# PABannier/bark.cpp

Hardware: NVIDIA H100
Metric: audio sec/sec (inverse RTF), bark-small f16, batch 1 per GPU, semantic->coarse->fine->encodec (higher is better)
Workload: dtype f16 weights/operands, f32 accumulate (reference arithmetic)

## Files before the change

### bark.cpp_b200/__init__.py

```python
from __future__ import annotations

import ctypes as C
import math
import os

import numpy as np

_HERE = os.path.dirname(os.path.abspath(__file__))
LIB_PATH = os.path.join(_HERE, "libbark_b200.so")

PROGRESS_CB = C.CFUNCTYPE(None, C.c_void_p, C.c_int, C.c_int, C.c_void_p)


class BarkContextParams(C.Structure):
    _fields_ = [
        ("verbosity", C.c_int), ("temp", C.c_float), ("fine_temp", C.c_float), ("min_eos_p", C.c_float),
        ("sliding_window_size", C.c_int32), ("max_coarse_history", C.c_int32), ("sample_rate", C.c_int32),
        ("target_bandwidth", C.c_int32), ("cls_token_id", C.c_int32), ("sep_token_id", C.c_int32),
        ("n_steps_text_encoder", C.c_int32), ("text_pad_token", C.c_int32), ("text_encoding_offset", C.c_int32),
        ("semantic_rate_hz", C.c_float), ("semantic_pad_token", C.c_int32), ("semantic_vocab_size", C.c_int32),
        ("semantic_infer_token", C.c_int32), ("coarse_rate_hz", C.c_float), ("coarse_infer_token", C.c_int32),
        ("coarse_semantic_pad_token", C.c_int32), ("n_coarse_codebooks", C.c_int32), ("n_fine_codebooks", C.c_int32),
        ("codebook_size", C.c_int32), ("progress_callback", PROGRESS_CB), ("progress_callback_user_data", C.c_void_p),
    ]
# ... 10 lines not shown

class HistoryPromptStruct(C.Structure):
    _fields_ = [("semantic", C.c_void_p), ("n_semantic", C.c_int), ("coarse", C.c_void_p), ("n_coarse_frames", C.c_int),
                ("fine", C.c_void_p), ("n_fine_frames", C.c_int)]


HISTORY_KEYS = ("semantic_prompt", "coarse_prompt", "fine_prompt")


def load_history_prompt(src) -> dict:
    if isinstance(src, (str, bytes, os.PathLike)):
        with np.load(src) as f:
            return load_history_prompt({k: f[k] for k in f.files})
    out = {}
    for k, lead in zip(HISTORY_KEYS, (None, 2, 8)):
        try:
            a = np.asarray(src[k])
        except KeyError:
            raise ValueError(f"history prompt: missing {k}") from None
        if a.dtype.kind not in "iu":
            raise ValueError(f"history prompt: {k} holds {a.dtype} values, not integer ids")
        if lead is None and a.ndim != 1:
            raise ValueError(f"history prompt: {k} has shape {a.shape}, expected [n]")
        if lead is not None and (a.ndim != 2 or a.shape[0] != lead):
            raise ValueError(f"history prompt: {k} has shape {a.shape}, expected [{lead}][n]")
        out[k] = np.ascontiguousarray(a, np.int32)
    return out


class SamplingStruct(C.Structure):
    _fields_ = [("top_k", C.c_int32), ("use_top_p", C.c_int32), ("top_p", C.c_float)]


SAMPLING_STAGES = {"semantic": 0, "coarse": 1}


def _sampling_struct(top_k=None, top_p=None):
    return SamplingStruct(int(top_k or 0), int(top_p is not None), float(top_p) if top_p is not None else 1.0)


def _history_struct(p):
    p = load_history_prompt(p)
    s, c, f = (p[k] for k in HISTORY_KEYS)
    return HistoryPromptStruct(_p(s), s.size, _p(c), c.shape[1], _p(f) if f.size else None, f.shape[1]), p


EXPORTS = [
    "bark_context_default_params", "bark_load_model", "bark_generate_audio", "bark_get_audio_data", "bark_get_audio_data_size",
    "bark_get_load_time", "bark_get_eval_time", "bark_reset_statistics", "bark_model_quantize", "bark_free",
    "bark_b200_set_device", "bark_b200_version", "bark_b200_gpt_eval", "bark_b200_fine_eval", "bark_b200_encodec_decode",
    "bark_b200_encodec_encode", "bark_b200_rvq_encode",
    "bark_b200_sample", "bark_b200_sample_rows", "bark_b200_reseed", "bark_b200_tokenize", "bark_b200_forward_text_encoder",
    "bark_b200_forward_coarse_encoder", "bark_b200_forward_fine_encoder", "bark_b200_get_tokens", "bark_b200_set_tokens",
    "bark_b200_get_stats", "bark_b200_get_hparams", "bark_b200_kernel_launches", "bark_b200_layernorm_fallbacks",
    "bark_b200_profile_enable", "bark_b200_profile_report", "bark_b200_io_counters", "bark_b200_decode_timing",
    "bark_b200_shard_init", "bark_b200_shard_connect", "bark_b200_shard_nvlink_bytes",
    "bark_b200_fast_mode", "bark_b200_fast_gemm", "bark_b200_fast_attention", "bark_b200_parity_attention", "bark_b200_batch_attention", "bark_b200_parity_gemm",
    "bark_b200_parity_rows", "bark_b200_sample_given_u", "bark_b200_generate_batch", "bark_b200_batch_audio", "bark_b200_batch_tokens", "bark_b200_gpt_eval_slot", "bark_b200_gpt_step_batch",
    "bark_b200_set_history_prompt", "bark_b200_generate_batch_prompted", "bark_b200_set_sampling", "bark_b200_sample_filtered_given_u",
    "bark_b200_quant_matmul", "bark_b200_fast_convert",
    "bark_b200_encodec_compress_batch", "bark_b200_encodec_decompress_batch", "bark_b200_encodec_reconstruct_batch",
    "bark_b200_encodec_batch_codes", "bark_b200_encodec_batch_audio",
    "bark_b200_encodec_compress_resampled", "bark_b200_encodec_reconstruct_resampled", "bark_b200_encodec_compress_batch_resampled",
    "bark_b200_encodec_reconstruct_batch_resampled", "bark_b200_encodec_encode_resampled", "bark_b200_resample",
    "ggml_time_init", "ggml_time_us", "ggml_time_ms", "ggml_init", "ggml_free",
]

ENCODEC_EXPORTS = [
    "encodec_load_model", "encodec_set_target_bandwidth", "encodec_set_sample_rate", "encodec_reconstruct_audio", "encodec_compress_audio",
    "encodec_decompress_audio", "encodec_get_audio", "encodec_get_audio_size", "encodec_get_codes", "encodec_get_codes_size",
    "encodec_get_statistics", "encodec_reset_statistics", "encodec_free",
]

_lib = None


def lib() -> C.CDLL:
    global _lib
    if _lib is not None:
        return _lib
    if not os.path.exists(LIB_PATH):
        raise RuntimeError(f"{LIB_PATH} is missing: build the CUDA extension first (python -c 'import __graft_entry__ as g; g.build()'). "
                           "There is no CPU fallback.")
    L = C.CDLL(LIB_PATH)
    vp, i32p, f32p = C.c_void_p, C.c_void_p, C.c_void_p
    L.bark_context_default_params.restype = BarkContextParams
    L.bark_load_model.restype = vp
    L.bark_load_model.argtypes = [C.c_char_p, BarkContextParams, C.c_uint32]
    L.bark_generate_audio.restype = C.c_bool
    L.bark_generate_audio.argtypes = [vp, C.c_char_p, C.c_int]
    L.bark_get_audio_data.restype = C.POINTER(C.c_float)
    L.bark_get_audio_data.argtypes = [vp]
    L.bark_get_audio_data_size.restype = C.c_int
    L.bark_get_audio_data_size.argtypes = [vp]
    for n in ("bark_get_load_time", "bark_get_eval_time"):
        getattr(L, n).restype = C.c_int64
        getattr(L, n).argtypes = [vp]
    L.bark_reset_statistics.argtypes = [vp]
    L.bark_model_quantize.restype = C.c_bool
    L.bark_model_quantize.argtypes = [C.c_char_p, C.c_char_p, C.c_int]
    L.bark_free.argtypes = [vp]
    L.bark_b200_set_device.argtypes = [C.c_int]
    L.bark_b200_version.restype = C.c_char_p
    L.bark_b200_gpt_eval.restype = C.c_int
    L.bark_b200_gpt_eval.argtypes = [vp, C.c_int, i32p, C.c_int, C.POINTER(C.c_int), C.c_int, f32p]
    L.bark_b200_fine_eval.restype = C.c_int
    L.bark_b200_fine_eval.argtypes = [vp, i32p, C.c_int, f32p]
    L.bark_b200_encodec_decode.restype = C.c_int
    L.bark_b200_encodec_decode.argtypes = [vp, i32p, C.c_int, f32p, C.c_int]
    L.bark_b200_encodec_encode.restype = C.c_int
    L.bark_b200_encodec_encode.argtypes = [vp, f32p, C.c_int, i32p, C.c_int, f32p, C.c_int]
    L.bark_b200_rvq_encode.restype = C.c_int
    L.bark_b200_rvq_encode.argtypes = [f32p, C.c_int, f32p, C.c_int, C.c_int, C.c_int, i32p]
    L.bark_b200_sample.restype = C.c_int
    L.bark_b200_sample.argtypes = [vp, C.c_int, f32p, C.c_int, C.c_float, C.POINTER(C.c_float)]
    L.bark_b200_sample_rows.restype = C.c_int
    L.bark_b200_sample_rows.argtypes = [vp, f32p, C.c_int, C.c_int, C.c_float, i32p, f32p]
    L.bark_b200_reseed.argtypes = [vp, C.c_uint32]
    L.bark_b200_tokenize.argtypes = [vp, C.c_char_p, i32p]
    for n in ("bark_b200_forward_text_encoder", "bark_b200_forward_coarse_encoder", "bark_b200_forward_fine_encoder"):
        getattr(L, n).restype = C.c_bool
        getattr(L, n).argtypes = [vp, C.c_int]
    L.bark_b200_get_tokens.restype = C.c_int
    L.bark_b200_get_tokens.argtypes = [vp, C.c_int, i32p, C.c_int]
    L.bark_b200_set_tokens.argtypes = [vp, C.c_int, i32p, C.c_int]
    L.bark_b200_get_stats.argtypes = [vp, C.POINTER(BarkStatistics), C.c_void_p]
    L.bark_b200_get_hparams.argtypes = [vp, C.c_int, i32p]
    L.bark_b200_kernel_launches.restype = C.c_ulonglong
    L.bark_b200_layernorm_fallbacks.restype = C.c_uint
    L.bark_b200_layernorm_fallbacks.argtypes = [vp]
    L.bark_b200_profile_enable.argtypes = [C.c_int]
    L.bark_b200_profile_report.restype = C.c_int
    L.bark_b200_profile_report.argtypes = [C.c_char_p, C.c_int]
    L.bark_b200_io_counters.argtypes = [C.POINTER(C.c_ulonglong), C.POINTER(C.c_ulonglong), C.c_int]
    L.bark_b200_decode_timing.restype = C.c_int
    L.bark_b200_decode_timing.argtypes = [vp, C.c_void_p, C.c_int]
    L.bark_b200_shard_init.restype = C.c_int
    L.bark_b200_shard_init.argtypes = [vp, C.c_int, C.c_int, vp]
    L.bark_b200_shard_connect.restype = C.c_int
    L.bark_b200_shard_connect.argtypes = [vp, vp]
    L.bark_b200_shard_nvlink_bytes.restype = C.c_ulonglong
    L.bark_b200_shard_nvlink_bytes.argtypes = [vp, C.c_int]
    L.bark_b200_fast_mode.restype = C.c_int
    L.bark_b200_fast_mode.argtypes = [vp]
    L.bark_b200_fast_gemm.restype = C.c_int
    L.bark_b200_fast_gemm.argtypes = [vp, vp, vp, C.c_int, C.c_int, C.c_int, C.c_int, C.c_int]
    L.bark_b200_fast_convert.restype = C.c_int
    L.bark_b200_fast_convert.argtypes = [C.c_int, vp, C.c_int, C.c_int, vp, C.POINTER(C.c_int)]
    L.bark_b200_fast_attention.restype = C.c_int
    L.bark_b200_fast_attention.argtypes = [vp, vp, vp, vp, C.c_int, C.c_int, C.c_int]
    L.bark_b200_parity_attention.restype = C.c_int
    L.bark_b200_parity_attention.argtypes = [vp, vp, vp, vp] + [C.c_int] * 7
    L.bark_b200_batch_attention.restype = C.c_int
    L.bark_b200_batch_attention.argtypes = [f32p, f32p, f32p, f32p, f32p, i32p] + [C.c_int] * 5 + [vp]
    L.bark_b200_parity_gemm.restype = C.c_int
    L.bark_b200_parity_gemm.argtypes = [vp, vp, vp] + [C.c_int] * 6 + [vp]
    L.bark_b200_quant_matmul.restype = C.c_int
    L.bark_b200_quant_matmul.argtypes = [C.c_int, vp, vp, vp] + [C.c_int] * 5 + [vp, vp, vp, vp]
    L.bark_b200_parity_rows.restype = C.c_int
    L.bark_b200_parity_rows.argtypes = [C.c_int, C.c_int, vp, C.c_int, C.c_int, vp, vp, vp, C.POINTER(C.c_uint)]
    L.bark_b200_sample_given_u.restype = C.c_int
    L.bark_b200_sample_given_u.argtypes = [f32p, C.c_int, C.c_int, C.c_float, vp, C.c_int, i32p, i32p, i32p, f32p]
    L.bark_b200_generate_batch.restype = C.c_bool
    L.bark_b200_generate_batch.argtypes = [vp, C.POINTER(C.c_char_p), C.POINTER(C.c_uint32), C.c_int, C.c_int]
    L.bark_b200_batch_audio.restype = C.c_int
    L.bark_b200_batch_audio.argtypes = [vp, C.c_int, f32p, C.c_int]
    L.bark_b200_batch_tokens.restype = C.c_int
    L.bark_b200_batch_tokens.argtypes = [vp, C.c_int, C.c_int, i32p, C.c_int]
    L.bark_b200_gpt_eval_slot.restype = C.c_int
    L.bark_b200_gpt_eval_slot.argtypes = [vp, C.c_int, C.c_int, i32p, C.c_int, C.POINTER(C.c_int), C.c_int, f32p]
    L.bark_b200_gpt_step_batch.restype = C.c_int
    L.bark_b200_gpt_step_batch.argtypes = [vp, C.c_int, C.c_int, i32p, i32p, i32p, f32p]
    L.bark_b200_set_sampling.restype = C.c_int
    L.bark_b200_set_sampling.argtypes = [vp, C.c_int, C.POINTER(SamplingStruct)]
    L.bark_b200_sample_filtered_given_u.restype = C.c_int
    L.bark_b200_sample_filtered_given_u.argtypes = [f32p, C.c_int, C.c_int, C.c_float, C.POINTER(SamplingStruct), vp, C.c_int, i32p, i32p, i32p, f32p, i32p]
    L.bark_b200_set_history_prompt.restype = C.c_int
    L.bark_b200_set_history_prompt.argtypes = [vp, C.POINTER(HistoryPromptStruct)]
    L.bark_b200_generate_batch_prompted.restype = C.c_bool
    L.bark_b200_generate_batch_prompted.argtypes = [vp, C.POINTER(C.c_char_p), C.POINTER(C.c_uint32), C.POINTER(C.POINTER(HistoryPromptStruct)),
                                                    C.c_int, C.c_int]
    for n in ("bark_b200_encodec_compress_batch", "bark_b200_encodec_decompress_batch", "bark_b200_encodec_reconstruct_batch"):
        getattr(L, n).restype = C.c_bool
# ... 613 lines not shown
            xs = self._batch_resampled("bark_b200_encodec_reconstruct_batch_resampled", clips, sample_rate)
        return [self._item("bark_b200_encodec_batch_audio", i, np.float32) for i in range(len(xs))]

    def _batch_resampled(self, fn, clips, sample_rate):
        fr = [_frames(a) for a in clips]
        n = len(fr)
        rates = [int(sample_rate)] * n if np.ndim(sample_rate) == 0 else [int(r) for r in sample_rate]
        if len(rates) != n:
            raise ValueError(f"{fn}: {n} clips but {len(rates)} sample rates")
        ptrs = (C.c_void_p * max(n, 1))(*[x.ctypes.data for x, _, _ in fr])
        frames = (C.c_int * max(n, 1))(*[nf for _, nf, _ in fr])
        chans = (C.c_int * max(n, 1))(*[ch for _, _, ch in fr])
        srs = (C.c_int * max(n, 1))(*rates)
        if not getattr(lib(), fn)(self.ctx, ptrs, frames, chans, srs, n):
            raise RuntimeError(f"{fn} failed (see stderr)")
        return [resampled_length(nf, r) for (_, nf, _), r in zip(fr, rates)]

    def _batch(self, fn, arrays):
        n = len(arrays)
        ptrs = (C.c_void_p * max(n, 1))(*[a.ctypes.data for a in arrays])
        lens = (C.c_int * max(n, 1))(*[a.size for a in arrays])
        if not getattr(lib(), fn)(self.ctx, ptrs, lens, n):
            raise RuntimeError(f"{fn} failed (see stderr)")

    def _item(self, fn, i, dtype):
        n = getattr(lib(), fn)(self.ctx, i, None, 0)
        out = np.empty(n, dtype)
        getattr(lib(), fn)(self.ctx, i, _p(out), n)
        return out

    def stats(self) -> dict:
        s = lib().encodec_get_statistics(self.ctx).contents
        return {"t_load_us": s.t_load_us, "t_compute_us": s.t_compute_us}

    def reset_stats(self):
        lib().encodec_reset_statistics(self.ctx)


def rvq_encode(latent: np.ndarray, codebooks: np.ndarray) -> np.ndarray:
    lat = np.ascontiguousarray(latent, np.float32); cb = np.ascontiguousarray(codebooks, np.float32)
    hidden, T = lat.shape
    n_q, n_bins, h2 = cb.shape
    assert h2 == hidden, (lat.shape, cb.shape)
    codes = np.zeros((n_q, T), np.int32)
    if not lib().bark_b200_rvq_encode(_p(lat), T, _p(cb), hidden, n_bins, n_q, _p(codes)):
        raise RuntimeError(f"bark_b200_rvq_encode ({hidden} x {T}, {n_q} x {n_bins} codewords) failed")
    return codes


def kernel_launches() -> int:
    return int(lib().bark_b200_kernel_launches())


def profile_enable(on: bool):
    lib().bark_b200_profile_enable(int(on))


def profile_report() -> dict:
    import json
    n = lib().bark_b200_profile_report(None, 0)
    buf = C.create_string_buffer(n + 16)
    lib().bark_b200_profile_report(buf, n + 16)
    return json.loads(buf.value.decode())


def io_counters(reset: bool = False):
    a, b = C.c_ulonglong(0), C.c_ulonglong(0)
    lib().bark_b200_io_counters(C.byref(a), C.byref(b), int(reset))
    return a.value, b.value
```

### bark.cpp_b200/csrc/bark_api.cu

```cuda
#include "../../include/bark_b200.h"
#include "context.h"
#include "codec_kernels.h"
#include "gpt_kernels.h"

#include <algorithm>
#include <cmath>
#include <cstring>
#include <stdexcept>

using namespace bark;

namespace {

thread_local int g_device_override = -1;
bool quiet() { static const bool q = [] { const char * e = getenv("BARK_B200_QUIET"); return e && *e && *e != '0'; }(); return q; }

inline bool is_alpha(unsigned char c) { return (c >= 'a' && c <= 'z') || (c >= 'A' && c <= 'Z'); }
inline bool is_digit(unsigned char c) { return c >= '0' && c <= '9'; }
inline bool is_punct(unsigned char c) { return c > 32 && c < 127 && !is_alpha(c) && !is_digit(c); }

char fold_accent(unsigned char second) {
    const unsigned cp = 0xC0u + (second - 0x80u);
    const bool lower = cp >= 0xE0;
    const unsigned up = lower ? cp - 0x20 : cp;
// ... 785 lines not shown
    const int64_t t0 = now_us();
    const double u = temp != 0.0f && n > 1 ? std::generate_canonical<double, 53>(ctx->gen.rng) : 0.0;
    const int32_t next = sample_token_given_u(logits, n, temp, u, eos_p);
    m.t_sample_us += now_us() - t0;
    m.n_sample += 1;
    return next;
}
static int bark_b200_sample_rows_impl(struct bark_context * ctx, const float * logits, int n, int rows, float temp, int32_t * tokens_out, float * eos_p_out) {
    if (!ctx || !logits || !tokens_out || rows < 1 || rows > 1024 || n < 2 || n > kSampleMaxLogits) return -1;
    const size_t cap = std::max<size_t>({(size_t) ctx->semantic.n_out_vocab, (size_t) ctx->coarse.n_out_vocab, (size_t) 1024 * ctx->fine.n_out_vocab});
    if ((size_t) rows * n > cap) return -1;
    BARK_CUDA_CHECK(cudaSetDevice(ctx->device));
    BARK_CUDA_CHECK(cudaMemcpyAsync(ctx->ws.logits, logits, (size_t) rows * n * 4, cudaMemcpyHostToDevice, ctx->stream));
    const long long before = ctx->n_sample_host_replays;
    if (!sample_device(ctx, ctx->fine, ctx->gen.rng, ctx->ws.logits, n, n, rows, temp, tokens_out, eos_p_out)) return -1;
    return (int)(ctx->n_sample_host_replays - before);
}
extern "C" int bark_b200_sample_rows(struct bark_context * ctx, const float * logits, int n, int rows, float temp, int32_t * tokens_out, float * eos_p_out) { return guarded((int) -1, [&] { return bark_b200_sample_rows_impl(ctx, logits, n, rows, temp, tokens_out, eos_p_out); }); }
extern "C" void bark_b200_reseed(struct bark_context * ctx, uint32_t seed) { if (ctx) ctx->gen.rng = std::mt19937(seed); }
extern "C" void bark_b200_tokenize(struct bark_context * ctx, const char * text, int32_t * out513) {
    if (!ctx || !text || !out513) return;
    tokenize_input(ctx, ctx->gen, text);
    memcpy(out513, ctx->gen.tokens.data(), sizeof(int32_t) * 513);
}
static int copy_tokens(const Generation & g, int stage, int32_t * out, int cap) {
    const std::vector<int32_t> * v = stage == 0 ? &g.semantic_tokens : stage == 1 ? &g.coarse_tokens : stage == 2 ? &g.fine_tokens : stage == 3 ? &g.tokens : nullptr;
    if (!v) return -1;
    if (out) memcpy(out, v->data(), sizeof(int32_t) * std::min(v->size(), (size_t) std::max(cap, 0)));
    return (int) v->size();
}
extern "C" int bark_b200_get_tokens(struct bark_context * ctx, int stage, int32_t * out, int cap) { return ctx ? copy_tokens(ctx->gen, stage, out, cap) : -1; }
extern "C" void bark_b200_set_tokens(struct bark_context * ctx, int stage, const int32_t * in, int n) {
    if (!ctx || !in || n < 0) return;
    Generation & g = ctx->gen;
    if (stage == 0) g.semantic_tokens.assign(in, in + n); else if (stage == 1) g.coarse_tokens.assign(in, in + n); else if (stage == 3) g.tokens.assign(in, in + n);
}
extern "C" void bark_b200_get_stats(struct bark_context * ctx, struct bark_statistics * out, int64_t * per_model9) {
    if (!ctx) return;
    if (out) *out = ctx->stats;
    if (per_model9) { const GPTModel * m[3] = {&ctx->semantic, &ctx->coarse, &ctx->fine}; for (int i = 0; i < 3; i++) { per_model9[3 * i] = m[i]->t_predict_us; per_model9[3 * i + 1] = m[i]->t_sample_us; per_model9[3 * i + 2] = m[i]->n_sample; } }
}
extern "C" void bark_b200_get_hparams(struct bark_context * ctx, int which, int32_t * out10) {
    if (!ctx || !out10) return;
    const GPTModel * m = pick(ctx, which); if (!m) return;
    const int32_t v[10] = {m->n_layer, m->n_head, m->n_embd, m->block_size, m->bias, m->n_in_vocab, m->n_out_vocab, m->n_lm_heads, m->n_wtes, m->ftype};
    memcpy(out10, v, sizeof(v));
}
extern "C" unsigned long long bark_b200_kernel_launches(void) { return g_kernel_launches.load(); }
static unsigned bark_b200_layernorm_fallbacks_impl(struct bark_context * ctx) {
    if (!ctx) return 0;
    unsigned v = 0; BARK_CUDA_CHECK(cudaMemcpy(&v, ctx->d_ln_fallbacks, sizeof(v), cudaMemcpyDeviceToHost)); return v;
}
extern "C" unsigned bark_b200_layernorm_fallbacks(struct bark_context * ctx) { return guarded((unsigned) 0, [&] { return bark_b200_layernorm_fallbacks_impl(ctx); }); }
static int bark_b200_decode_timing_impl(struct bark_context * ctx, unsigned long long * out, int n) {
    if (!ctx || !ctx->d_timing || !out) return 0;
    BARK_CUDA_CHECK(cudaMemcpy(out, ctx->d_timing, sizeof(unsigned long long) * (size_t) std::min(n, 256 * 32), cudaMemcpyDeviceToHost));
    return std::min(n, 256 * 32);
}
extern "C" int bark_b200_decode_timing(struct bark_context * ctx, unsigned long long * out, int n) { return guarded((int) 0, [&] { return bark_b200_decode_timing_impl(ctx, out, n); }); }
extern "C" int bark_b200_fast_mode(struct bark_context * ctx) { return ctx && ctx->fast_mode ? 1 : 0; }

extern "C" int bark_b200_set_sampling(struct bark_context * ctx, int stage, const struct bark_b200_sampling * s) {
    const char * fn = "bark_b200_set_sampling";
    if (!ctx) { fprintf(stderr, "%s: invalid bark context\n", fn); return 0; }
    if (stage != 0 && stage != 1) { fprintf(stderr, "%s: stage %d (0 semantic, 1 coarse; the fine stage has no filter)\n", fn, stage); return 0; }
    if (s && !sampling_valid(fn, *s)) return 0;
    ctx->sampling[stage] = s ? *s : bark_b200_sampling{0, 0, 1.0f};
    return 1;
}

extern "C" bool bark_b200_generate_batch(struct bark_context * ctx, const char * const * texts, const uint32_t * seeds, int n, int n_threads) {
    (void) n_threads;
    return guarded(false, [&] { return generate_batch(ctx, texts, seeds, nullptr, n); });
}
extern "C" bool bark_b200_generate_batch_prompted(struct bark_context * ctx, const char * const * texts, const uint32_t * seeds,
                                                  const struct bark_b200_history_prompt * const * prompts, int n, int n_threads) {
    (void) n_threads;
    return guarded(false, [&] { return generate_batch(ctx, texts, seeds, prompts, n); });
}
extern "C" int bark_b200_set_history_prompt(struct bark_context * ctx, const struct bark_b200_history_prompt * prompt) {
    if (!ctx) { fprintf(stderr, "bark_b200_set_history_prompt: invalid bark context\n"); return 0; }
    return guarded((int) 0, [&] {
        HistoryPrompt h;
        if (prompt && !make_history_prompt(ctx->params, *prompt, h)) return 0;
        ctx->gen.prompt = std::move(h);
        return 1;
    });
}
extern "C" int bark_b200_batch_audio(struct bark_context * ctx, int i, float * out, int cap) {
    if (!ctx || i < 0 || i >= (int) ctx->batch.results.size()) return -1;
    const std::vector<float> & a = ctx->batch.results[(size_t) i].audio;
    if (out) memcpy(out, a.data(), sizeof(float) * std::min(a.size(), (size_t) std::max(cap, 0)));
    return (int) a.size();
}
extern "C" int bark_b200_batch_tokens(struct bark_context * ctx, int i, int stage, int32_t * out, int cap) {
    if (!ctx || i < 0 || i >= (int) ctx->batch.results.size()) return -1;
    return copy_tokens(ctx->batch.results[(size_t) i], stage, out, cap);
}
static int bark_b200_gpt_eval_slot_impl(struct bark_context * ctx, int which, int slot, const int32_t * tokens, int n, int * n_past, int merge_ctx, float * logits_out) {
    if (!ctx || which < 0 || which > 1 || slot < 0 || slot >= kMaxBatch || !tokens || !n_past || !logits_out) return 0;
    BARK_CUDA_CHECK(cudaSetDevice(ctx->device));
    if (!ensure_batch_slots(ctx, slot + 1)) return 0;
    return gpt_eval(ctx, *pick(ctx, which), tokens, n, n_past, merge_ctx != 0, logits_out, 0, 0, ctx->batch.k[which][slot], ctx->batch.v[which][slot]) ? 1 : 0;
}
extern "C" int bark_b200_gpt_eval_slot(struct bark_context * ctx, int which, int slot, const int32_t * tokens, int n, int * n_past, int merge_ctx, float * logits_out) {
    return guarded((int) 0, [&] { return bark_b200_gpt_eval_slot_impl(ctx, which, slot, tokens, n, n_past, merge_ctx, logits_out); });
// ... 27 lines not shown
```

### bark.cpp_b200/csrc/context.h

```cpp
#pragma once
#include "../../include/bark_b200.h"
#include "gpt_kernels.h"

#include <fstream>
#include <map>
#include <random>
#include <string>
#include <vector>

struct ShardState {
    bool on = false; int rank = 0, world = 1;
    unsigned char * local = nullptr, * peer[8] = {nullptr};
    unsigned epoch = 0; unsigned * d_err = nullptr;
    unsigned long long nvlink_bytes = 0;
};

struct HistoryPrompt {
    std::vector<int32_t> semantic;
    std::vector<int32_t> coarse;
    std::vector<int32_t> fine;
    bool empty() const { return semantic.empty(); }
};

struct Generation {
// ... 52 lines not shown
    int32_t * h_tok = nullptr;

    bark::CodecScratch codec_scratch;

    Generation gen;
    BatchSlots batch;

    bark_context_params params;
    bark_statistics stats{};

    bark::DeviceArena arena;
};

namespace bark {

bool load_model_file(const std::string & path, bark_context * ctx);
void * ctx_alloc(bark_context * ctx, size_t bytes);

bool gpt_eval(bark_context * ctx, GPTModel & m, const int32_t * tokens, int n, int * n_past, bool merge_ctx, float * logits_host, int lm_lo = 0, int lm_hi = 0,
              float * mem_k = nullptr, float * mem_v = nullptr);
bool gpt_step_batch(bark_context * ctx, GPTModel & m, int B, float * const * slot_k, float * const * slot_v, const int32_t * tokens, const int * n_past,
                    int lm_lo, int lm_hi, float * d_logits);
void build_decode_tables(bark_context * ctx, GPTModel & m);
bool fine_eval(bark_context * ctx, const int32_t * in_buffer , int nn, float * logits_host );
bool fine_eval_shard(bark_context * ctx, const int32_t * in_buffer, int nn);
bool sample_shard(bark_context * ctx, std::mt19937 & rng, int n, float temp, int32_t * out_all );
bool fine_eval_fast(bark_context * ctx, const int32_t * in_buffer, int nn, float * logits_host);
bool gpt_decode_chained(bark_context * ctx, GPTModel & m, const int32_t * d_token, int * n_past, int lm_lo, int lm_hi);
bool fine_embed(bark_context * ctx, const int32_t * in_buffer, int nn, int row0, int rows, const char * fn);
void output_head(bark_context * ctx, const GPTModel & m, const float * x, int rows, const DMat & head, float * logits, int lo = 0);

struct ActLayout { WType wt; int kpE, kp4E; };
template <class KV> void run_layers(bark_context * ctx, const GPTModel & m, int rows, const KV & kv);
struct ShardKV {
    int row0;
    void store(bark_context * ctx, const GPTModel & m, int il, int rows, MatmulEpilogue & qkv) const;
    void attend(bark_context * ctx, const GPTModel & m, int il, int rows, const ActLayout & a) const;
};
bool load_codec(std::ifstream & f, CodecModel & c, int max_q, DeviceArena & arena, cudaStream_t s, bool verbose);
constexpr int kCodecLaunchFrames = 24000;
bool codec_decode(const CodecModel & cm, CodecScratch & sc, cudaStream_t s, int n, const int32_t * const * codes, const int * T, int n_q,
                  std::vector<float> * audio, const char * batch_fn = nullptr);
struct CodecOutputs { std::vector<int32_t> * codes = nullptr; std::vector<float> * latent = nullptr, * audio = nullptr; };
constexpr int kCodecSampleRate = 24000;
struct AudioFormat { int channels, sample_rate; };
bool codec_encode(const CodecModel & cm, CodecScratch & sc, cudaStream_t s, int n, const float * const * audio, const int * n_samples, int n_q,
                  const CodecOutputs & out, const char * batch_fn = nullptr, const AudioFormat * fmt = nullptr);
bool resample_input_ok(const char * fn, const std::string & item, const float * x, int n_frames, int channels, int sample_rate);
std::string item_tag(const char * batch_fn, int i);

constexpr int kSampleMaxLogits = 16384;
void sample_rows(const float * logits, int ld, int n, int rows, float temp, const double * d_u, int32_t * d_out_tok, int tok_add, int32_t * d_feed,
                 float * d_eos_p, int32_t * d_flags, int force_flag, int threads, cudaStream_t s);
int32_t sample_token_given_u(const float * logits, int n, float temp, double u, float * eos_p);
inline bool filter_on(const bark_b200_sampling & f) { return f.top_k > 0 || f.use_top_p != 0; }
bool sampling_valid(const char * fn, const bark_b200_sampling & s);
constexpr int kMaxFilterRows = 8;
void filter_rows(const float * logits, int ld, int n, int rows, const bark_b200_sampling & f, float * d_out, int32_t * d_kept, int32_t * d_flags, int threads,
                 cudaStream_t s);
int filter_row_host(float * row, int n, const bark_b200_sampling & f);
void read_back_samples(bark_context * ctx, int start, int stop, bool want_eos, bool filtered);
inline bool sample_flagged(const bark_context * ctx, int r, bool filtered) { return ctx->h_sflags[r] || (filtered && ctx->h_fflags[r]); }
int sample_and_replay(bark_context * ctx, const float * d_logits, int ld, int lo, int n, int rows, float temp, bool want_eos, const bark_b200_sampling * f = nullptr);
bool sample_device(bark_context * ctx, GPTModel & m, std::mt19937 & rng, const float * d_logits, int ld, int n, int rows, float temp, int32_t * out_tok, float * out_eos);

int64_t now_us();
int select_device(const char * caller, cudaDeviceProp * prop);

}
```

### bark.cpp_b200/csrc/sampling.cu

```cuda
#include "context.h"
#include "gpt_kernels.h"

#include <algorithm>
#include <cmath>
#include <stdexcept>

namespace bark {

template <int kSampleThreads>
__device__ __forceinline__ void sample_row_body(float * sh, const float * lg, int n, float temp, double u, int32_t * out_tok, int tok_add, int32_t * feed,
                                                float * eos_p, int32_t * flags, int force_flag) {
    __shared__ float s_f[kSampleThreads / 32]; __shared__ int s_i[kSampleThreads / 32]; __shared__ double s_d[kSampleThreads / 32];
    __shared__ float s_sum; __shared__ int s_amb;
    const int tid = threadIdx.x, lane = tid & 31, warp = tid >> 5;
    constexpr int NW = kSampleThreads / 32;
    const float div = temp == 0.0f ? 0.7f : temp;
    bool ambiguous = force_flag != 0;
    if (tid == 0) s_amb = 0;

    float mx = __int_as_float(0xff800000);
    for (int i = tid; i < n; i += kSampleThreads) { const float l = __fdiv_rn(__ldcg(lg + i), div); sh[i] = l; mx = fmaxf(mx, l); }
#pragma unroll
    for (int o = 16; o > 0; o >>= 1) mx = fmaxf(mx, __shfl_xor_sync(0xffffffffu, mx, o));
    if (lane == 0) s_f[warp] = mx;
    __syncthreads();
    mx = s_f[0];
#pragma unroll
    for (int w = 1; w < NW; w++) mx = fmaxf(mx, s_f[w]);
    for (int i = tid; i < n; i += kSampleThreads) {
        const double y = exp((double) __fsub_rn(sh[i], mx));
        if (__double2float_rn(y * (1.0 - 0x1p-50)) != __double2float_rn(y * (1.0 + 0x1p-50))) ambiguous = true;
        sh[i] = __double2float_rn(y);
    }
    __syncthreads();
    if (tid == 0) {
        float sum = 0.0f;
        int i = 0;
        for (; i + 8 <= n; i += 8) {
            const float4 a = *reinterpret_cast<const float4 *>(sh + i), b = *reinterpret_cast<const float4 *>(sh + i + 4);
            sum = __fadd_rn(sum, a.x); sum = __fadd_rn(sum, a.y); sum = __fadd_rn(sum, a.z); sum = __fadd_rn(sum, a.w);
            sum = __fadd_rn(sum, b.x); sum = __fadd_rn(sum, b.y); sum = __fadd_rn(sum, b.z); sum = __fadd_rn(sum, b.w);
        }
        for (; i < n; i++) sum = __fadd_rn(sum, sh[i]);
        s_sum = sum;
    }
    __syncthreads();
    const float sum = s_sum;
    for (int i = tid; i < n; i += kSampleThreads) sh[i] = __fdiv_rn(sh[i], sum);
    __syncthreads();

    int token = 0;
    if (temp == 0.0f) {
        float best = __int_as_float(0xff800000); int bi = 0x7fffffff;
        for (int i = tid; i < n; i += kSampleThreads) { const float p = sh[i]; if (p > best) { best = p; bi = i; } }
#pragma unroll
        for (int o = 16; o > 0; o >>= 1) {
            const float ob = __shfl_xor_sync(0xffffffffu, best, o); const int oi = __shfl_xor_sync(0xffffffffu, bi, o);
            if (ob > best || (ob == best && oi < bi)) { best = ob; bi = oi; }
        }
        if (lane == 0) { s_f[warp] = best; s_i[warp] = bi; }
        __syncthreads();
        best = s_f[0]; bi = s_i[0];
#pragma unroll
        for (int w = 1; w < NW; w++) if (s_f[w] > best || (s_f[w] == best && s_i[w] < bi)) { best = s_f[w]; bi = s_i[w]; }
        token = bi;
    } else {
        const int c = (n + kSampleThreads - 1) / kSampleThreads, lo = min(n, tid * c), hi = min(n, lo + c);
        double part = 0.0;
        for (int i = lo; i < hi; i++) part += (double) sh[i];
        double incl = part;
#pragma unroll
        for (int o = 1; o < 32; o <<= 1) { const double t = __shfl_up_sync(0xffffffffu, incl, o); if (lane >= o) incl += t; }
        if (lane == 31) s_d[warp] = incl;
        __syncthreads();
        double before = 0.0, total = 0.0;
#pragma unroll
        for (int w = 0; w < NW; w++) { if (w < warp) before += s_d[w]; total += s_d[w]; }
        const double thr = u * total;
        const double eps = 8.0 * (double) n * 0x1p-53 * total;
        double run = before + incl - part;
        int first = 0x7fffffff;
        for (int i = lo; i < hi; i++) {
            run += (double) sh[i];
            if (i < n - 1) {
                if (fabs(run - thr) <= eps) ambiguous = true;
                if (run >= thr && first == 0x7fffffff) first = i;
            }
        }
#pragma unroll
        for (int o = 16; o > 0; o >>= 1) first = min(first, __shfl_xor_sync(0xffffffffu, first, o));
        if (lane == 0) s_i[warp] = first;
        __syncthreads();
        first = s_i[0];
#pragma unroll
        for (int w = 1; w < NW; w++) first = min(first, s_i[w]);
        token = first == 0x7fffffff ? n - 1 : first;
    }
    if (ambiguous) s_amb = 1;
    __syncthreads();
    if (tid == 0) {
        *out_tok = token + tok_add;
        if (feed) *feed = token + tok_add;
        if (eos_p) *eos_p = sh[n - 1];
        *flags = s_amb;
    }
}

template <int kSampleThreads>
__global__ void __launch_bounds__(kSampleThreads) sample_rows_kernel(const float * __restrict__ logits, int ld, int n, int rows, float temp, const double * __restrict__ u,
                                                                     int32_t * __restrict__ out_tok, int tok_add, int32_t * __restrict__ feed,
                                                                     float * __restrict__ eos_p, int32_t * __restrict__ flags, int force_flag) {
    extern __shared__ float sh[];
    const int row = blockIdx.x;
    sample_row_body<kSampleThreads>(sh, logits + (size_t) row * ld, n, temp, temp != 0.0f ? u[row] : 0.0, out_tok + row, tok_add, feed ? feed + row : nullptr,
                                    eos_p ? eos_p + row : nullptr, flags + row, force_flag);
}

void sample_rows(const float * logits, int ld, int n, int rows, float temp, const double * d_u, int32_t * d_out_tok, int tok_add, int32_t * d_feed,
                 float * d_eos_p, int32_t * d_flags, int force_flag, int threads, cudaStream_t s) {
    const size_t smem = ((size_t) n * sizeof(float) + 15) & ~(size_t) 15;
    static std::atomic<unsigned long long> configured{0};
    if (first_use_on_this_device(configured)) {
        BARK_CUDA_CHECK(cudaFuncSetAttribute(sample_rows_kernel<256>, cudaFuncAttributeMaxDynamicSharedMemorySize, kSampleMaxLogits * (int) sizeof(float)));
        BARK_CUDA_CHECK(cudaFuncSetAttribute(sample_rows_kernel<1024>, cudaFuncAttributeMaxDynamicSharedMemorySize, kSampleMaxLogits * (int) sizeof(float)));
    }
    if (threads == 0) threads = rows == 1 ? 1024 : 256;
    g_next_bytes = (double) rows * n * 4.0;
    if (threads == 1024) BARK_LAUNCH(sample_rows_kernel<1024>, rows, 1024, smem, s, logits, ld, n, rows, temp, d_u, d_out_tok, tok_add, d_feed, d_eos_p, d_flags, force_flag);
    else                 BARK_LAUNCH(sample_rows_kernel<256>, rows, 256, smem, s, logits, ld, n, rows, temp, d_u, d_out_tok, tok_add, d_feed, d_eos_p, d_flags, force_flag);
}

__device__ __forceinline__ unsigned long long filter_key(float x, int i) {
    const unsigned b = x == 0.0f ? 0u : __float_as_uint(x);
    return (unsigned long long)((b & 0x80000000u) ? ~b : (b | 0x80000000u)) << 32 | (unsigned) i;
}
__device__ __forceinline__ float filter_key_value(unsigned long long k) {
    const unsigned o = (unsigned)(k >> 32);
    return __uint_as_float((o & 0x80000000u) ? (o & 0x7fffffffu) : ~o);
}

template <int kThreads>
__global__ void __launch_bounds__(kThreads, 1) filter_rows_kernel(const float * __restrict__ logits, int ld, int n, int P, int top_k, int use_top_p, float top_p,
                                                               float * __restrict__ out, int32_t * __restrict__ kept, int32_t * __restrict__ flags) {
    extern __shared__ unsigned long long sk[];
    float * e = reinterpret_cast<float *>(sk + P);
    __shared__ int s_amb, s_K, s_L, s_cnt; __shared__ float s_sum;
    const int tid = threadIdx.x;
    const float * lg = logits + (size_t) blockIdx.x * ld;
    if (tid == 0) { s_amb = 0; s_cnt = 0; }
    bool amb = false;
    for (int i = tid; i < P; i += kThreads) {
        if (i < n) { const float x = __ldcg(lg + i); if (x != x) amb = true; sk[i] = filter_key(x, i); }
        else sk[i] = 0ull;
    }
    __syncthreads();
    for (int k = 2; k <= P; k <<= 1)
        for (int j = k >> 1; j > 0; j >>= 1) {
            for (int t = tid; t < P / 2; t += kThreads) {
                const int a = 2 * t - (t & (j - 1)), b = a + j;
                const unsigned long long ka = sk[a], kb = sk[b];
                if ((a & k) == 0 ? ka < kb : ka > kb) { sk[a] = kb; sk[b] = ka; }
            }
            __syncthreads();
        }
    const float m = filter_key_value(sk[0]);
    if (!isfinite(m)) amb = true;
    int Kp = n;
    if (use_top_p) {
// ... 194 lines not shown
```

### include/bark_b200.h

```cpp
#pragma once
#include "bark.h"

#ifdef __cplusplus
extern "C" {
#endif

BARK_API void bark_b200_set_device(int cuda_device);
BARK_API const char * bark_b200_version(void);

BARK_API int  bark_b200_gpt_eval(struct bark_context * ctx, int which, const int32_t * tokens, int n, int * n_past, int merge_ctx, float * logits_out);
BARK_API int  bark_b200_fine_eval(struct bark_context * ctx, const int32_t * in_buffer, int nn, float * logits_out);
BARK_API int  bark_b200_encodec_decode(struct bark_context * ctx, const int32_t * codes, int n_frames, float * out, int out_cap);
BARK_API int  bark_b200_encodec_encode(struct bark_context * ctx, const float * audio, int n_samples, int32_t * codes, int codes_cap,
                                       float * latent, int latent_cap);
BARK_API int  bark_b200_rvq_encode(const float * latent, int T, const float * codebooks, int hidden, int n_bins, int n_q, int32_t * codes);
BARK_API int  bark_b200_sample(struct bark_context * ctx, int which, const float * logits, int n, float temp, float * eos_p);
BARK_API int  bark_b200_sample_rows(struct bark_context * ctx, const float * logits , int n, int rows, float temp, int32_t * tokens_out,
                                     float * eos_p_out );
BARK_API void bark_b200_reseed(struct bark_context * ctx, uint32_t seed);
BARK_API void bark_b200_tokenize(struct bark_context * ctx, const char * text, int32_t * out513);

BARK_API bool bark_b200_forward_text_encoder(struct bark_context * ctx, int n_threads);
BARK_API bool bark_b200_forward_coarse_encoder(struct bark_context * ctx, int n_threads);
BARK_API bool bark_b200_forward_fine_encoder(struct bark_context * ctx, int n_threads);

BARK_API int  bark_b200_get_tokens(struct bark_context * ctx, int stage, int32_t * out, int cap);
BARK_API void bark_b200_set_tokens(struct bark_context * ctx, int stage, const int32_t * in, int n);
BARK_API void bark_b200_get_stats(struct bark_context * ctx, struct bark_statistics * out, int64_t * per_model9);
BARK_API void bark_b200_get_hparams(struct bark_context * ctx, int which, int32_t * out10);
BARK_API unsigned long long bark_b200_kernel_launches(void);
BARK_API unsigned bark_b200_layernorm_fallbacks(struct bark_context * ctx);

BARK_API void bark_b200_profile_enable(int on);
BARK_API int  bark_b200_profile_report(char * buf, int cap);
BARK_API void bark_b200_io_counters(unsigned long long * h2d_bytes, unsigned long long * d2h_bytes, int reset);
BARK_API int  bark_b200_decode_timing(struct bark_context * ctx, unsigned long long * out, int n);


BARK_API int  bark_b200_shard_init(struct bark_context * ctx, int rank, int world, void * handle_out);
BARK_API int  bark_b200_shard_connect(struct bark_context * ctx, const void * all_handles);
BARK_API unsigned long long bark_b200_shard_nvlink_bytes(struct bark_context * ctx, int reset);

BARK_API bool bark_b200_generate_batch(struct bark_context * ctx, const char * const * texts, const uint32_t * seeds, int n, int n_threads);
BARK_API int  bark_b200_batch_audio(struct bark_context * ctx, int i, float * out, int cap);
BARK_API int  bark_b200_batch_tokens(struct bark_context * ctx, int i, int stage, int32_t * out, int cap);
BARK_API int  bark_b200_gpt_eval_slot(struct bark_context * ctx, int which, int slot, const int32_t * tokens, int n, int * n_past, int merge_ctx, float * logits_out);
BARK_API int  bark_b200_gpt_step_batch(struct bark_context * ctx, int which, int B, const int32_t * slots, const int32_t * tokens, int * n_past, float * logits_out);

struct bark_b200_history_prompt {
    const int32_t * semantic; int n_semantic;
    const int32_t * coarse;   int n_coarse_frames;
    const int32_t * fine;     int n_fine_frames;
};
BARK_API int  bark_b200_set_history_prompt(struct bark_context * ctx, const struct bark_b200_history_prompt * prompt);
BARK_API bool bark_b200_generate_batch_prompted(struct bark_context * ctx, const char * const * texts, const uint32_t * seeds,
                                                const struct bark_b200_history_prompt * const * prompts, int n, int n_threads);

struct bark_b200_sampling {
    int32_t top_k;
    int32_t use_top_p;
    float   top_p;
};
BARK_API int  bark_b200_set_sampling(struct bark_context * ctx, int stage, const struct bark_b200_sampling * s);
BARK_API int  bark_b200_sample_filtered_given_u(const float * logits, int n, int rows, float temp, const struct bark_b200_sampling * s,
                                                const double * u, int threads, int32_t * tokens, int32_t * device_tokens, int32_t * flags,
                                                float * eos_p, int32_t * kept);

#define BARK_B200_ENCODEC_MAX_BATCH 1024
BARK_API bool bark_b200_encodec_compress_batch(struct encodec_context * e, const float * const * audio, const int * n_samples, int n);
BARK_API bool bark_b200_encodec_decompress_batch(struct encodec_context * e, const int32_t * const * codes, const int * n_codes, int n);
BARK_API bool bark_b200_encodec_reconstruct_batch(struct encodec_context * e, const float * const * audio, const int * n_samples, int n);
BARK_API int  bark_b200_encodec_batch_codes(struct encodec_context * e, int i, int32_t * out, int cap);
BARK_API int  bark_b200_encodec_batch_audio(struct encodec_context * e, int i, float * out, int cap);

BARK_API bool bark_b200_encodec_compress_resampled(struct encodec_context * e, const float * audio, int n_frames, int channels, int sample_rate);
BARK_API bool bark_b200_encodec_reconstruct_resampled(struct encodec_context * e, const float * audio, int n_frames, int channels, int sample_rate);
BARK_API bool bark_b200_encodec_compress_batch_resampled(struct encodec_context * e, const float * const * audio, const int * n_frames, const int * channels,
                                                         const int * sample_rates, int n);
BARK_API bool bark_b200_encodec_reconstruct_batch_resampled(struct encodec_context * e, const float * const * audio, const int * n_frames, const int * channels,
                                                            const int * sample_rates, int n);
BARK_API int  bark_b200_encodec_encode_resampled(struct bark_context * ctx, const float * audio, int n_frames, int channels, int sample_rate, int32_t * codes,
                                                 int codes_cap, float * latent, int latent_cap);
BARK_API int  bark_b200_resample(const float * in, int n_frames, int channels, int in_rate, int out_rate, float * out, int cap);

// ... 26 lines not shown
```

Measured before the change: 13.18.

## Parallelize sequential softmax sum in sampler with speculative piecewise float chains

Replaces the single-thread sequential float summation of exponentiated logits, used for bit-exact softmax normalization, with a per-warp piecewise scheme for rows of 2048 or more. Each warp computes its chunk's chain from 32 candidate starting values near a double-precision estimate of the prefix, then the true chain is stitched together via shuffles. A fallback recomputes serially when the guess misses, counted in a new device counter. This removes a long serial loop per sampling step in the semantic and coarse stages, at the cost of more arithmetic and shared memory.

```diff
diff --git a/bark.cpp_b200/__init__.py b/bark.cpp_b200/__init__.py
--- a/bark.cpp_b200/__init__.py
+++ b/bark.cpp_b200/__init__.py
@@ -86,7 +86,7 @@
     "bark_b200_encodec_encode", "bark_b200_rvq_encode",
     "bark_b200_sample", "bark_b200_sample_rows", "bark_b200_reseed", "bark_b200_tokenize", "bark_b200_forward_text_encoder",
     "bark_b200_forward_coarse_encoder", "bark_b200_forward_fine_encoder", "bark_b200_get_tokens", "bark_b200_set_tokens",
-    "bark_b200_get_stats", "bark_b200_get_hparams", "bark_b200_kernel_launches", "bark_b200_layernorm_fallbacks",
+    "bark_b200_get_stats", "bark_b200_get_hparams", "bark_b200_kernel_launches", "bark_b200_layernorm_fallbacks", "bark_b200_sample_misses",
     "bark_b200_profile_enable", "bark_b200_profile_report", "bark_b200_io_counters", "bark_b200_decode_timing",
     "bark_b200_shard_init", "bark_b200_shard_connect", "bark_b200_shard_nvlink_bytes",
     "bark_b200_fast_mode", "bark_b200_fast_gemm", "bark_b200_fast_attention", "bark_b200_parity_attention", "bark_b200_batch_attention", "bark_b200_parity_gemm",
@@ -163,6 +163,7 @@
     L.bark_b200_kernel_launches.restype = C.c_ulonglong
     L.bark_b200_layernorm_fallbacks.restype = C.c_uint
     L.bark_b200_layernorm_fallbacks.argtypes = [vp]
+    L.bark_b200_sample_misses.restype = C.c_uint
     L.bark_b200_profile_enable.argtypes = [C.c_int]
     L.bark_b200_profile_report.restype = C.c_int
     L.bark_b200_profile_report.argtypes = [C.c_char_p, C.c_int]
@@ -882,6 +883,10 @@
     return int(lib().bark_b200_kernel_launches())
 
 
+def sample_misses() -> int:
+    return int(lib().bark_b200_sample_misses())
+
+
 def profile_enable(on: bool):
     lib().bark_b200_profile_enable(int(on))
 
diff --git a/bark.cpp_b200/csrc/bark_api.cu b/bark.cpp_b200/csrc/bark_api.cu
--- a/bark.cpp_b200/csrc/bark_api.cu
+++ b/bark.cpp_b200/csrc/bark_api.cu
@@ -861,6 +861,7 @@
     unsigned v = 0; BARK_CUDA_CHECK(cudaMemcpy(&v, ctx->d_ln_fallbacks, sizeof(v), cudaMemcpyDeviceToHost)); return v;
 }
 extern "C" unsigned bark_b200_layernorm_fallbacks(struct bark_context * ctx) { return guarded((unsigned) 0, [&] { return bark_b200_layernorm_fallbacks_impl(ctx); }); }
+extern "C" unsigned bark_b200_sample_misses(void) { return guarded((unsigned) 0, [&] { return sample_misses(); }); }
 static int bark_b200_decode_timing_impl(struct bark_context * ctx, unsigned long long * out, int n) {
     if (!ctx || !ctx->d_timing || !out) return 0;
     BARK_CUDA_CHECK(cudaMemcpy(out, ctx->d_timing, sizeof(unsigned long long) * (size_t) std::min(n, 256 * 32), cudaMemcpyDeviceToHost));
diff --git a/bark.cpp_b200/csrc/context.h b/bark.cpp_b200/csrc/context.h
--- a/bark.cpp_b200/csrc/context.h
+++ b/bark.cpp_b200/csrc/context.h
@@ -128,6 +128,7 @@
 constexpr int kSampleMaxLogits = 16384;
 void sample_rows(const float * logits, int ld, int n, int rows, float temp, const double * d_u, int32_t * d_out_tok, int tok_add, int32_t * d_feed,
                  float * d_eos_p, int32_t * d_flags, int force_flag, int threads, cudaStream_t s);
+unsigned sample_misses();
 int32_t sample_token_given_u(const float * logits, int n, float temp, double u, float * eos_p);
 inline bool filter_on(const bark_b200_sampling & f) { return f.top_k > 0 || f.use_top_p != 0; }
 bool sampling_valid(const char * fn, const bark_b200_sampling & s);
diff --git a/bark.cpp_b200/csrc/sampling.cu b/bark.cpp_b200/csrc/sampling.cu
--- a/bark.cpp_b200/csrc/sampling.cu
+++ b/bark.cpp_b200/csrc/sampling.cu
@@ -7,13 +7,37 @@
 
 namespace bark {
 
+__device__ unsigned g_sample_misses;
+
+__device__ __forceinline__ float float_chain(float s, const float * x, int len) {
+    int i = 0;
+    for (; i + 8 <= len; i += 8) {
+        const float4 a = *reinterpret_cast<const float4 *>(x + i), b = *reinterpret_cast<const float4 *>(x + i + 4);
+        s = __fadd_rn(s, a.x); s = __fadd_rn(s, a.y); s = __fadd_rn(s, a.z); s = __fadd_rn(s, a.w);
+        s = __fadd_rn(s, b.x); s = __fadd_rn(s, b.y); s = __fadd_rn(s, b.z); s = __fadd_rn(s, b.w);
+    }
+    for (; i < len; i++) s = __fadd_rn(s, x[i]);
+    return s;
+}
+
+__device__ __forceinline__ double warp_exclusive_sum(double v) {
+    const int lane = threadIdx.x & 31;
+#pragma unroll
+    for (int o = 1; o < 32; o <<= 1) { const double t = __shfl_up_sync(0xffffffffu, v, o); if (lane >= o) v += t; }
+    const double before = __shfl_up_sync(0xffffffffu, v, 1);
+    return lane == 0 ? 0.0 : before;
+}
+
 template <int kSampleThreads>
 __device__ __forceinline__ void sample_row_body(float * sh, const float * lg, int n, float temp, double u, int32_t * out_tok, int tok_add, int32_t * feed,
                                                 float * eos_p, int32_t * flags, int force_flag) {
-    __shared__ float s_f[kSampleThreads / 32]; __shared__ int s_i[kSampleThreads / 32]; __shared__ double s_d[kSampleThreads / 32];
+    constexpr int NW = kSampleThreads / 32;
+    constexpr int P = NW, C = 32;
+    constexpr int kPieceMinRow = 2048;
+    __shared__ float s_f[NW]; __shared__ int s_i[NW]; __shared__ double s_d[NW];
+    __shared__ float s_end1[P], s_end2[P][C]; __shared__ unsigned char s_next[P][C];
     __shared__ float s_sum; __shared__ int s_amb;
     const int tid = threadIdx.x, lane = tid & 31, warp = tid >> 5;
-    constexpr int NW = kSampleThreads / 32;
     const float div = temp == 0.0f ? 0.7f : temp;
     bool ambiguous = force_flag != 0;
     if (tid == 0) s_amb = 0;
@@ -27,25 +51,62 @@
     mx = s_f[0];
 #pragma unroll
     for (int w = 1; w < NW; w++) mx = fmaxf(mx, s_f[w]);
-    for (int i = tid; i < n; i += kSampleThreads) {
+    const bool pieces = n >= kPieceMinRow;
+    const int L = ((n + P - 1) / P + 7) & ~7, lo = min(n, warp * L), hi = min(n, lo + L);
+    double part = 0.0;
+    for (int i = pieces ? lo + lane : tid; i < (pieces ? hi : n); i += pieces ? 32 : kSampleThreads) {
         const double y = exp((double) __fsub_rn(sh[i], mx));
         if (__double2float_rn(y * (1.0 - 0x1p-50)) != __double2float_rn(y * (1.0 + 0x1p-50))) ambiguous = true;
-        sh[i] = __double2float_rn(y);
-    }
-    __syncthreads();
-    if (tid == 0) {
-        float sum = 0.0f;
-        int i = 0;
-        for (; i + 8 <= n; i += 8) {
-            const float4 a = *reinterpret_cast<const float4 *>(sh + i), b = *reinterpret_cast<const float4 *>(sh + i + 4);
-            sum = __fadd_rn(sum, a.x); sum = __fadd_rn(sum, a.y); sum = __fadd_rn(sum, a.z); sum = __fadd_rn(sum, a.w);
-            sum = __fadd_rn(sum, b.x); sum = __fadd_rn(sum, b.y); sum = __fadd_rn(sum, b.z); sum = __fadd_rn(sum, b.w);
-        }
-        for (; i < n; i++) sum = __fadd_rn(sum, sh[i]);
-        s_sum = sum;
-    }
-    __syncthreads();
-    const float sum = s_sum;
+        const float e = __double2float_rn(y);
+        sh[i] = e; part += (double) e;
+    }
+    float sum;
+    if (!pieces) {
+        __syncthreads();
+        if (tid == 0) s_sum = float_chain(0.0f, sh, n);
+        __syncthreads();
+        sum = s_sum;
+    } else {
+#pragma unroll
+        for (int o = 16; o > 0; o >>= 1) part += __shfl_xor_sync(0xffffffffu, part, o);
+        if (lane == 0) s_d[warp] = part;
+        __syncthreads();
+        const float g = __double2float_rn(warp_exclusive_sum(lane < P ? s_d[lane] : 0.0));
+        const float gp = __shfl_sync(0xffffffffu, g, warp);
+        if (lane == 0) s_end1[warp] = float_chain(gp, sh + lo, hi - lo);
+        __syncthreads();
+        const float h = __double2float_rn(warp_exclusive_sum(lane < P ? (double) s_end1[lane] - (double) g : 0.0));
+        const unsigned hp = __float_as_uint(__shfl_sync(0xffffffffu, h, warp));
+        const float end = float_chain(__uint_as_float(hp + lane - C / 2), sh + lo, hi - lo);
+        const unsigned next = __float_as_uint(end) - __float_as_uint(__shfl_sync(0xffffffffu, h, (warp + 1) & 31)) + C / 2;
+        s_end2[warp][lane] = end;
+        s_next[warp][lane] = next < (unsigned) C ? next : C;
+        __syncthreads();
+        unsigned o = C / 2;
+#pragma unroll
+        for (int p = 0; p < P - 1; p++) {
+            const unsigned m = s_next[p][lane];
+            if (o < (unsigned) C) o = __shfl_sync(0xffffffffu, m, o);
+        }
+        if (o < (unsigned) C) {
+            sum = s_end2[P - 1][o];
+        } else {
+            if (warp == 0) {
+                float s = 0.0f;
+                for (int p = 0; p < P; p++) {
+                    const unsigned j = __float_as_uint(s) - __float_as_uint(__shfl_sync(0xffffffffu, h, p)) + C / 2;
+                    if (j < (unsigned) C) s = s_end2[p][j];
+                    else if (p * L < n) {
+                        s = float_chain(s, sh + p * L, min(n, p * L + L) - p * L);
+                        if (lane == 0) atomicAdd(&g_sample_misses, 1u);
+                    }
+                }
+                if (lane == 0) s_sum = s;
+            }
+            __syncthreads();
+            sum = s_sum;
+        }
+    }
     for (int i = tid; i < n; i += kSampleThreads) sh[i] = __fdiv_rn(sh[i], sum);
     __syncthreads();
 
@@ -114,6 +175,12 @@
     const int row = blockIdx.x;
     sample_row_body<kSampleThreads>(sh, logits + (size_t) row * ld, n, temp, temp != 0.0f ? u[row] : 0.0, out_tok + row, tok_add, feed ? feed + row : nullptr,
                                     eos_p ? eos_p + row : nullptr, flags + row, force_flag);
+}
+
+unsigned sample_misses() {
+    unsigned v = 0;
+    BARK_CUDA_CHECK(cudaMemcpyFromSymbol(&v, g_sample_misses, sizeof(v)));
+    return v;
 }
 
 void sample_rows(const float * logits, int ld, int n, int rows, float temp, const double * d_u, int32_t * d_out_tok, int tok_add, int32_t * d_feed,
diff --git a/include/bark_b200.h b/include/bark_b200.h
--- a/include/bark_b200.h
+++ b/include/bark_b200.h
@@ -30,6 +30,7 @@
 BARK_API void bark_b200_get_hparams(struct bark_context * ctx, int which, int32_t * out10);
 BARK_API unsigned long long bark_b200_kernel_launches(void);
 BARK_API unsigned bark_b200_layernorm_fallbacks(struct bark_context * ctx);
+BARK_API unsigned bark_b200_sample_misses(void);
 
 BARK_API void bark_b200_profile_enable(int on);
 BARK_API int  bark_b200_profile_report(char * buf, int cap);
```

Result: no change. 13.25 (median of 6 runs) (+0.6%).
